# Illumina/Pisces

Hardware: AMD Instinct MI355X
Metric: candidate loci/s at 500x depth (higher is better)
Workload: dtype int32 counts + f64 likelihoods; 1 GPU; BASELINE config 2: synthetic 100000 loci x 500x amplicon pileup, SNV-only, gVCF, per GPU per step; device-resident packed tuples; depth=500, ring_batches=6, tile_loci=56, parallelism=interval-shard x1

## Files before the change

### pisces_amd/csrc/store_kernels.hip.h

```cpp
#pragma once
#include <hip/hip_runtime.h>
#include <stdint.h>
#include <type_traits>

#include "kernels.hip.h"
#include "read_walk.h"
#include "stream_kernels.hip.h"

#ifndef PISCES_ADD_OCC
#define PISCES_ADD_OCC 6
#endif
#ifdef PISCES_ADD_STAMPS
#define PISCES_STAMP(k, is_max) do { if (threadIdx.x == 0) A.stamps[(long long)blockIdx.x * 8 + ((k) == 0 ? 2 : (k) == 1 ? 3 : (k) - 2)] = (long long)wall_clock64(); } while (0)
#else
#define PISCES_STAMP(k, is_max) do { } while (0)
#endif
namespace pisces {

struct ReadDesc {
    int32_t pos0;
    uint32_t meta;
    int64_t aoff;
};
struct ReadExt {
    int64_t cig_off;
    int32_t n_cigar;
    int32_t n_bases;
};
static_assert(sizeof(ReadDesc) == 16 && sizeof(ReadExt) == 16, "descriptor layout");
constexpr uint32_t kDescLenMask = 0xFFFFFu;
constexpr uint32_t kDescComplex = 1u << 20;
constexpr uint32_t kDescReverse = 1u << 21;
constexpr uint32_t kDescGeneric = 1u << 22;
// ... 101 lines not shown
            const long long a = prev + 1, b = p;
            if (b - a > kGridGapCells || b - A.grid_base >= A.grid_n || a < A.grid_base) atomicOr(&A.state[kStateFrags], kGridBadBit);
            else { c0 = (int)(a - A.grid_base); c1 = (int)(b - A.grid_base); f0 = (int)(A.ops0 + A.cigar_offset[r]); }
        }
    }
    const bool wide = c1 - c0 >= 16;
    if (!wide)
        for (int k = c0; k <= c1; k++) A.grid[k] = f0;
    for (unsigned long long m = __ballot(wide); m != 0ull; m &= m - 1ull) {
        const int src = __builtin_ctzll(m);
        const int b0 = __builtin_amdgcn_readlane(c0, src), b1 = __builtin_amdgcn_readlane(c1, src), f = __builtin_amdgcn_readlane(f0, src);
        for (int k = b0 + lane; k <= b1; k += 64) A.grid[k] = f;
    }
    if (block == (A.n_reads - 1) / 256) {
        const int last_lane = (A.n_reads - 1) & 255;
        if ((int)(threadIdx.x >> 6) == (last_lane >> 6)) {
            const long long p_last = A.position[A.n_reads - 1];
            const long long from = max(p_last + 1 - (long long)A.grid_base, 0ll);
            for (long long k = from + lane; k < (long long)A.grid_n; k += 64) A.grid[k] = 0x7F7F7F7F;
        }
    }
}

__device__ __forceinline__ void shape_reads(const ShapeArgs& A, const int block, const bool ok)
{
    const int r = block * 256 + (int)threadIdx.x;
    int reach = 0;
    bool unsorted = false, complex_read = false, generic_read = false, has_del = false;
    if (r < A.n_reads && ok) {
        const int c0 = A.cigar_offset[r], nc = A.cigar_offset[r + 1] - c0;
        const int s0 = A.seq_offset[r], n = A.seq_offset[r + 1] - s0;
        const int32_t pos0 = A.position[r];
        int phase = 0, lead = 0;
        long long run = 0, ref_span = 0;
        bool simple = true, prev_gap = false, gap_chain = false;
        for (int c = 0; c < nc; c++) {
            const uint8_t t = A.cigar_op[c0 + c];
            const long long len = A.cigar_len[c0 + c];
            if (walk_op_ref_span(t)) ref_span += len;
            if (t == 'D' || t == 'N') { gap_chain = gap_chain || prev_gap; prev_gap = true; }
            if (t == 'M' || t == '=' || t == 'X') {
                prev_gap = false;
                if (phase == 2) simple = false;
                phase = 1;
                run += len;
            } else if (t == 'S') {
                if (phase == 0) lead += (int)len;
                else phase = 2;
            } else if (t == 'H' || t == 'P') {
                if (phase == 1 && t == 'H') phase = 2;
            } else {
                simple = false;
            }
        }
        if (run > (long long)kDescLenMask || run > n - lead) simple = false;
        ReadDesc d;
        d.pos0 = pos0;
        d.meta = (simple ? (uint32_t)run : kDescComplex) | ((A.flags[r] & 1) ? kDescReverse : 0u);
        d.aoff = A.base0 + s0 + (simple ? lead : 0);
        A.desc[A.n0 + r] = d;
        ReadExt e;
        e.cig_off = A.ops0 + c0;
        e.n_cigar = nc;
        e.n_bases = n;
        A.ext[A.n0 + r] = e;
        reach = (int)(ref_span > 0x7FFFFFFFll ? 0x7FFFFFFFll : ref_span);
        complex_read = !simple;
        bool generic = ref_span > 0xFFFFll || gap_chain;
        const long long span16 = (ref_span > 0 ? ref_span - 1 : 0) << kFragSpanShift;
        for (int c = 0; c < nc; c++) generic = generic || A.cigar_len[c0 + c] > kDescLenMask;
        if (generic) {
            d.meta |= kDescGeneric;
            A.desc[A.n0 + r] = d;
        }
        const uint8_t* const quals = A.quals + s0;
        const uint32_t rev = (A.flags[r] & 1) ? kDescReverse : 0u;
        auto dq = [&](int i) {
            const int after = quals[i], before = i > 0 ? quals[i - 1] : after;
            return before >= A.min_bq && after >= A.min_bq;
        };
        auto dir_at = [&](int i) { return A.dirs ? (uint32_t)A.dirs[s0 + i] : (rev ? (uint32_t)PISCES_DIR_REVERSE : (uint32_t)PISCES_DIR_FORWARD); };
        const bool ends_in_del = nc >= 1 && A.cigar_op[c0 + nc - 1] == 'D';
        const bool ends_in_del_soft = nc >= 2 && A.cigar_op[c0 + nc - 2] == 'D' && A.cigar_op[c0 + nc - 1] == 'S';
        int ri = 0;
        long long rp = pos0, last_mapped = (long long)pos0 - 1;
        for (int c = 0; c < nc; c++) {
            const uint8_t t = A.cigar_op[c0 + c];
            const int len = (int)A.cigar_len[c0 + c];
            ReadDesc f;
            f.pos0 = pos0;
            f.meta = rev;
            f.aoff = A.base0 + s0;
            if (!generic && len > 0) {
                if (t == 'M' || t == '=' || t == 'X') {
                    const int have = max(min(len, n - ri), 0);
                    f.meta |= (uint32_t)have;
                    f.aoff = (A.base0 + s0 + ri) | span16 | ((rp - pos0) << kFragDeltaShift);
                } else if (t == 'D' || t == 'N') {
                    int idx = -1, first = (int)(rp - pos0), count = len;
                    uint32_t dir = 0;
                    {
                        int rj = ri;
                        for (int k = c + 1; k < nc && idx < 0; k++) {
                            const uint8_t tk = A.cigar_op[c0 + k];
                            const int lk = (int)A.cigar_len[c0 + k];
                            if ((tk == 'M' || tk == '=' || tk == 'X') && lk > 0) idx = rj;
                            else if (walk_op_read_span(tk)) rj += lk;
                        }
                    }
                    bool counted = false, terminal = false;
                    if (idx >= 0 && idx < n) {
                        counted = dq(idx);
                        dir = dir_at(idx);
                    } else if (t == 'D' && c == nc - 1 && ends_in_del && n > 0) {
                        counted = dq(n - 1);
                        dir = dir_at(n - 1);
                        first = (int)(last_mapped + 1 - pos0);
                        terminal = true;
                    } else if (t == 'D' && c == nc - 2 && ends_in_del_soft) {
                        const int at = n - (int)A.cigar_len[c0 + nc - 1];
                        if (at >= 0 && at < n) {
                            counted = dq(at);
                            dir = dir_at(at);
                            first = (int)(last_mapped + 1 - pos0);
                            terminal = true;
                        }
                    }
                    if (counted && first >= 0 && first <= 0xFFFF) {
                        f.meta = rev | kFragDeletion | (uint32_t)count | (dir << kFragDirShift) | (terminal ? kFragTerminal : 0u);
                        f.aoff = (A.base0 + s0) | span16 | ((long long)first << kFragDeltaShift);
                        has_del = true;
                    }
                }
            }
            A.frag[A.ops0 + c0 + c] = f;
            if (walk_op_ref_span(t)) {
                if (walk_op_read_span(t) && len > 0) last_mapped = rp + len - 1;
                rp += len;
            }
            if (walk_op_read_span(t)) ri += len;
        }
        generic_read = generic;
        if (r > 0) unsorted = A.position[r - 1] > pos0;
        else if (A.n0 > 0) unsorted = A.desc[A.n0 - 1].pos0 > pos0;
    }
#pragma unroll
    for (int d = 32; d >= 1; d >>= 1) reach = max(reach, __shfl_xor(reach, d, 64));
    const bool any_unsorted = __ballot(unsorted) != 0ull, any_complex = __ballot(complex_read) != 0ull;
    const int frag_bits = (__ballot(generic_read) != 0ull ? 1 : 0) | (__ballot(has_del) != 0ull ? 2 : 0);
    if ((threadIdx.x & 63) == 0) {
        if (reach > A.state[kStateReach]) atomicMax(&A.state[kStateReach], reach);
        if (any_unsorted && A.state[kStateUnsorted] == 0) atomicOr(&A.state[kStateUnsorted], 1);
        if (any_complex && A.state[kStateComplex] == 0) atomicOr(&A.state[kStateComplex], 1);
        if (frag_bits & ~A.state[kStateFrags]) atomicOr(&A.state[kStateFrags], frag_bits);
    }
}
__global__ __launch_bounds__(256) void read_shape_kernel(ShapeArgs A)
{
    if ((int)blockIdx.x >= A.shape_blocks) {
        const int b = (int)blockIdx.x - A.shape_blocks;
        if (b < A.enc_blocks) encode_rows(A, b, A.enc_blocks);
        else grid_cells(A, b - A.enc_blocks);
        return;
    }
    shape_reads(A, (int)blockIdx.x, true);
}

enum { kPrepPositionNotPositive = 1, kPrepMalformed = 2, kPrepCigarMismatch = 3, kPrepPastInt32 = 4, kPrepBadDeletionDirection = 5, kPrepBadDirection = 6 };
struct PrepareArgs {
    const int32_t* position;
    const int32_t* cigar_offset;
    const uint8_t* cigar_op;
    const uint32_t* cigar_len;
    const int32_t* seq_offset;
    const uint8_t* quals;
    const uint8_t* del_dirs;
    int32_t n_reads, min_bq, block_size, count_indels;
    int64_t n_ops_total, n_bases_total;
    uint32_t* block_bits;
    int64_t n_block_bits;
    int64_t map_stride;
    int32_t* n_found;
    int32_t* n_pool;
    unsigned long long* first_error;
    int32_t* key_span;
};
constexpr int kPrepReplicas = 32;
__device__ __forceinline__ void set_keys(const PrepareArgs& A, int replica, int64_t a, int64_t b)
{
    uint32_t* const map = A.block_bits + (int64_t)(replica & (kPrepReplicas - 1)) * A.map_stride;
    for (int64_t k = a; k <= b; k++) {
        if (k >= A.n_block_bits) continue;
        const uint32_t bit = 1u << (k & 31);
        uint32_t* const w = &map[k >> 5];
        (void)__hip_atomic_fetch_or(w, bit, __ATOMIC_RELAXED, __HIP_MEMORY_SCOPE_AGENT);
    }
}
__device__ __forceinline__ long long prep_shfl64(long long v, int src_lane)
{
    const int lo = __shfl((int)(v & 0xFFFFFFFFll), src_lane, 64);
    const int hi = __shfl((int)(v >> 32), src_lane, 64);
    return ((long long)hi << 32) | (unsigned int)lo;
}
__device__ __forceinline__ void prepare_reads(const PrepareArgs& A, const int block, int& found_out, int& pool_out, bool& ok_out)
{
    constexpr int kRunSlots = 32;
    __shared__ int s_klo, s_khi, s_plo, s_eqx, s_nruns;
    __shared__ long long s_run_a[kRunSlots], s_run_b[kRunSlots];
    if (threadIdx.x == 0) { s_klo = 0x7FFFFFFF; s_khi = 0; s_plo = 0x7FFFFFFF; s_eqx = 0; s_nruns = 0; }
    __syncthreads();
    const int r = block * 256 + (int)threadIdx.x;
    found_out = pool_out = 0;
    ok_out = false;
    int k_lo = 0x7FFFFFFF, k_hi = 0, p_lo = 0x7FFFFFFF;
    int64_t run_a = 1, run_b = 0;
    bool eqx = false;
    if (r < A.n_reads) {
        int code = 0;
        p_lo = A.position[r];
        const int64_t c0 = A.cigar_offset[r], c1 = A.cigar_offset[r + 1], s0 = A.seq_offset[r], s1 = A.seq_offset[r + 1];
        const int32_t pos0 = A.position[r];
        const int64_t nc = c1 - c0, n = s1 - s0;
        int found = 0, pool = 0;
        if (c0 < 0 || c1 < c0 || c1 > A.n_ops_total || s0 < 0 || s1 < s0 || s1 > A.n_bases_total) code = kPrepMalformed;
        else if (pos0 <= 0) code = kPrepPositionNotPositive;
        if (!code) {
            const uint8_t* const quals = A.quals + s0;
            auto delq = [&](int64_t idx) {
                if (n == 0) return false;
                const int after = idx < n ? quals[idx] : quals[idx - 1];
                const int before = idx > 0 ? quals[idx - 1] : after;
                return before >= A.min_bq && after >= A.min_bq;
            };
            auto touch = [&](int64_t from, int64_t to) {
                if (to < 1) return;
                if (from < 1) from = 1;
                const int64_t a = (from + A.block_size - 1) / A.block_size, b = (to + A.block_size - 1) / A.block_size;
                if (run_b < run_a) { run_a = a; run_b = b; }
                else if (a <= run_b + 1 && b >= run_a - 1) { run_a = min(run_a, a); run_b = max(run_b, b); }
                else { set_keys(A, block, run_a, run_b); run_a = a; run_b = b; }
                k_lo = min(k_lo, (int)a);
                k_hi = max(k_hi, (int)min(b, (int64_t)0x7FFFFFFF));
            };
            int64_t read_span = 0, ref_span = 0;
            bool bad_del_dir = false;
            for (int64_t c = 0; c < nc && !code; c++) {
                const uint8_t t = A.cigar_op[c0 + c];
                const uint32_t len = A.cigar_len[c0 + c];
                if (len > 0x0FFFFFFFu) code = kPrepMalformed;
                if (walk_op_read_span(t)) read_span += len;
                if (walk_op_ref_span(t)) ref_span += len;
                if (A.del_dirs && t == 'D')
                    for (int k = 0; k < 2; k++) {
                        const uint8_t d = A.del_dirs[2 * (c0 + c) + k];
                        if (d > 2 && d != PISCES_DIR_UNTRACKED) bad_del_dir = true;
                    }
                if (A.count_indels) {
                    if (t == 'I' || t == 'D') found++;
                    if (t == 'I' && len > 32u) pool += (int)len;
                    if (t == 'X' || t == '=') eqx = true;
                }
            }
            if (!code && nc > 0 && read_span != n) code = kPrepCigarMismatch;
            if (!code && (int64_t)pos0 + ref_span > 0x7FFFFFFFll) code = kPrepPastInt32;
            if (!code && bad_del_dir) code = kPrepBadDeletionDirection;
            if (!code) {
                int64_t rp = pos0, last_mapped = (int64_t)pos0 - 1, ri = 0;
                for (int64_t c = 0; c < nc; c++) {
                    const uint8_t t = A.cigar_op[c0 + c];
                    const int64_t len = A.cigar_len[c0 + c];
                    if (walk_op_read_span(t) && walk_op_ref_span(t) && len > 0) {
                        if (rp > last_mapped + 1 && ri < n && delq(ri)) touch(last_mapped + 1, rp - 1);
                        touch(rp, rp + len - 1);
                        last_mapped = rp + len - 1;
                    }
                    if (walk_op_ref_span(t)) rp += len;
                    if (walk_op_read_span(t)) ri += len;
                }
                const bool ends_del = nc >= 1 && A.cigar_op[c0 + nc - 1] == 'D';
                const bool ends_del_soft = nc >= 2 && A.cigar_op[c0 + nc - 2] == 'D' && A.cigar_op[c0 + nc - 1] == 'S';
                if (ends_del && n > 0 && delq(n - 1)) touch(last_mapped + 1, last_mapped + (int64_t)A.cigar_len[c0 + nc - 1]);
                if (ends_del_soft) {
                    const int64_t idx = n - (int64_t)A.cigar_len[c0 + nc - 1];
                    if (idx >= 0 && idx < n && delq(idx)) touch(last_mapped + 1, last_mapped + (int64_t)A.cigar_len[c0 + nc - 2]);
                }
            }
        }
        found_out = code ? 0 : found;
        pool_out = code ? 0 : pool;
        ok_out = code == 0;
        if (code) atomicMin(A.first_error, (unsigned long long)r * 8ull + (unsigned long long)code);
    }
    {
        unsigned long long todo = __ballot(run_b >= run_a);
        const int lane = threadIdx.x & 63;
        while (todo) {
            const int l0 = __builtin_ctzll(todo);
            const long long a0 = prep_shfl64((long long)run_a, l0), b0 = prep_shfl64((long long)run_b, l0);
            const unsigned long long same = __ballot(run_b >= run_a && run_a == a0 && run_b == b0);
            if (lane == l0) {
                const int slot = atomicAdd(&s_nruns, 1);
                if (slot < kRunSlots) { s_run_a[slot] = a0; s_run_b[slot] = b0; }
                else set_keys(A, block, a0, b0);
            }
            todo &= ~same;
        }
    }
#pragma unroll
    for (int d = 32; d >= 1; d >>= 1) {
        k_lo = min(k_lo, __shfl_xor(k_lo, d, 64));
        k_hi = max(k_hi, __shfl_xor(k_hi, d, 64));
        p_lo = min(p_lo, __shfl_xor(p_lo, d, 64));
    }
    const bool any_eqx = __ballot(eqx) != 0ull;
// ... 101 lines not shown
    int32_t do_shape;
    int32_t read_blocks, stream_blocks, misc_blocks;
    const uint8_t* s_bases;
    const uint8_t* s_quals;
    const uint8_t* s_dirs;
    uint8_t* d_bases;
    uint8_t* d_quals;
    uint8_t* d_dirs;
    uint8_t* d_codes;
    int64_t n_seq;
    uint32_t enc_min_bq;
    CopyRanges16 C;
    unsigned long long* scan_state;
    unsigned int* done;
    long long* totals;
    PrepVerdict* verdict;
    int32_t* keys_out;
    int32_t capacity;
    int32_t* bad_direction;
    int32_t seq;
    long long* stamps;
};
constexpr int kAddCopiedWord = 1;
__device__ __forceinline__ void wave_wait_vmem() { asm volatile("s_waitcnt vmcnt(0)" ::: "memory"); }
constexpr int kScanDirectBlocks = 4096;
constexpr unsigned long long kScanAggregate = 1ull << 62, kScanInclusive = 2ull << 62, kScanField = 0x7FFFFFFFull;

__device__ __forceinline__ void add_stream_roles(const AddFusedArgs& A, const int sb)
{
        if (sb < A.stream_blocks) {
            PISCES_STAMP(0, false);
            const uint32_t qk4 = (0x7Fu + A.enc_min_bq) * 0x01010101u;
            const int64_t n16 = A.n_seq >> 4;
            bool bad_dir = false;
            constexpr int kStreamPieces = 4;
            for (int64_t i0 = (int64_t)sb * (256 * kStreamPieces); i0 < n16; i0 += (int64_t)A.stream_blocks * (256 * kStreamPieces)) {
                uint32_t bw[kStreamPieces][4], qw[kStreamPieces][4];
#pragma unroll
                for (int p = 0; p < kStreamPieces; p++) {
                    const int64_t i = min(i0 + p * 256 + (int64_t)threadIdx.x, n16 - 1);
                    __builtin_memcpy(bw[p], A.s_bases + 16 * i, 16);
                    __builtin_memcpy(qw[p], A.s_quals + 16 * i, 16);
                }
#pragma unroll
                for (int p = 0; p < kStreamPieces; p++) {
                    const int64_t i = i0 + p * 256 + (int64_t)threadIdx.x;
                    if (i >= n16) continue;
                    if (A.s_dirs) {
                        uint32_t dw[4];
                        __builtin_memcpy(dw, A.s_dirs + 16 * i, 16);
#pragma unroll
                        for (int k = 0; k < 4; k++) bad_dir = bad_dir || ((dw[k] + 0x7D7D7D7Du) | dw[k]) & 0x80808080u;
                        if (A.d_dirs) __builtin_memcpy(A.d_dirs + 16 * i, dw, 16);
                    }
                    if (A.d_bases) {
                        __builtin_memcpy(A.d_bases + 16 * i, bw[p], 16);
                        __builtin_memcpy(A.d_quals + 16 * i, qw[p], 16);
                    }
// ... 38 lines not shown
    if (b >= A.read_blocks) {
        add_stream_roles(A, b - A.read_blocks);
        if (A.d_bases && !A.s_dirs) {
            wave_wait_vmem();
            __syncthreads();
            if (threadIdx.x == 0) {
                unsigned int* const copied = A.done + (1 + kPrepReplicas);
                const unsigned sb = (unsigned)(b - A.read_blocks), n_wg = (unsigned)(A.stream_blocks + A.misc_blocks);
                const unsigned cls = sb & (kPrepReplicas - 1u);
                const unsigned members = (n_wg - cls + kPrepReplicas - 1u) / kPrepReplicas;
                if (__hip_atomic_fetch_add(&copied[1 + cls], 1u, __ATOMIC_RELAXED, __HIP_MEMORY_SCOPE_AGENT) == members - 1u) {
                    __hip_atomic_store(&copied[1 + cls], 0u, __ATOMIC_RELAXED, __HIP_MEMORY_SCOPE_AGENT);
                    const unsigned classes = min(n_wg, (unsigned)kPrepReplicas);
                    if (__hip_atomic_fetch_add(&copied[0], 1u, __ATOMIC_RELAXED, __HIP_MEMORY_SCOPE_AGENT) == classes - 1u) {
                        __hip_atomic_store(&copied[0], 0u, __ATOMIC_RELAXED, __HIP_MEMORY_SCOPE_AGENT);
                        __hip_atomic_store(&A.bad_direction[kAddCopiedWord], A.seq, __ATOMIC_RELAXED, __HIP_MEMORY_SCOPE_SYSTEM);
                    }
                }
            }
        }
        return;
    }
    {
    int found, pool;
    bool ok;
    PISCES_STAMP(2, false);
    PISCES_STAMP(3, true);
    prepare_reads(A.P, b, found, pool, ok);
    PISCES_STAMP(4, true);
    if (A.do_shape) shape_reads(A.S, b, ok);
    PISCES_STAMP(5, true);
    const int lane = threadIdx.x & 63, wave = threadIdx.x >> 6;
    int incl_f = found, incl_p = pool;
#pragma unroll
    for (int d = 1; d < 64; d <<= 1) {
        const int uf = __shfl_up(incl_f, d, 64), up = __shfl_up(incl_p, d, 64);
        if (lane >= d) { incl_f += uf; incl_p += up; }
    }
    if (lane == 63) { s_wf[wave] = incl_f; s_wp[wave] = incl_p; }
    __syncthreads();
    int off_f = 0, off_p = 0, agg_f = 0, agg_p = 0;
#pragma unroll
    for (int w = 0; w < 4; w++) {
        if (w < wave) { off_f += s_wf[w]; off_p += s_wp[w]; }
        agg_f += s_wf[w]; agg_p += s_wp[w];
    }
    if (wave == 0) {
        const unsigned long long mine = ((unsigned long long)(unsigned)agg_p << 31) | (unsigned long long)(unsigned)agg_f;
        long long excl_f = 0, excl_p = 0;
        if (A.read_blocks <= kScanDirectBlocks) {
            if (lane == 0) __hip_atomic_store(&A.scan_state[b], kScanAggregate | mine, __ATOMIC_RELAXED, __HIP_MEMORY_SCOPE_AGENT);
            for (int i0 = 0; i0 < b; i0 += 64 * 16) {
                unsigned long long w[16];
                for (;;) {
                    bool all = true;
// ... 25 lines not shown
                if (none & upto) { __builtin_amdgcn_s_sleep(1); continue; }
                int f = (lane <= first_incl) ? (int)(w & kScanField) : 0, p = (lane <= first_incl) ? (int)((w >> 31) & kScanField) : 0;
#pragma unroll
                for (int d = 32; d >= 1; d >>= 1) { f += __shfl_xor(f, d, 64); p += __shfl_xor(p, d, 64); }
                excl_f += f; excl_p += p;
                if (first_incl < 64) break;
                base -= 64;
            }
            if (lane == 0)
                __hip_atomic_store(&A.scan_state[b], kScanInclusive | ((unsigned long long)(excl_p + agg_p) << 31) | (unsigned long long)(excl_f + agg_f), __ATOMIC_RELAXED,
                                   __HIP_MEMORY_SCOPE_AGENT);
        }
        if (lane == 0) {
            s_excl[0] = (int)excl_f; s_excl[1] = (int)excl_p;
            if (b == A.read_blocks - 1) {
                __hip_atomic_store(&A.totals[0], excl_f + agg_f, __ATOMIC_RELAXED, __HIP_MEMORY_SCOPE_AGENT);
                __hip_atomic_store(&A.totals[1], excl_p + agg_p, __ATOMIC_RELAXED, __HIP_MEMORY_SCOPE_AGENT);
            }
        }
    }
    __syncthreads();
    PISCES_STAMP(6, true);
    if (A.P.n_found) {
        const int r = b * 256 + (int)threadIdx.x;
        if (r < A.P.n_reads) {
            A.P.n_found[r] = s_excl[0] + off_f + incl_f - found;
            A.P.n_pool[r] = s_excl[1] + off_p + incl_p - pool;
        }
        if (b == A.read_blocks - 1 && threadIdx.x == 0) { A.P.n_found[A.P.n_reads] = s_excl[0] + agg_f; A.P.n_pool[A.P.n_reads] = s_excl[1] + agg_p; }
    }
    }
    wave_wait_vmem();
    __syncthreads();
    if (threadIdx.x == 0) {
        const unsigned cls = (unsigned)b & (kPrepReplicas - 1u);
        const unsigned members = ((unsigned)A.read_blocks - cls + kPrepReplicas - 1u) / kPrepReplicas;
        int last = 0;
        if (__hip_atomic_fetch_add(&A.done[1 + cls], 1u, __ATOMIC_RELAXED, __HIP_MEMORY_SCOPE_AGENT) == members - 1u) {
            const unsigned classes = min((unsigned)A.read_blocks, (unsigned)kPrepReplicas);
            last = __hip_atomic_fetch_add(&A.done[0], 1u, __ATOMIC_RELAXED, __HIP_MEMORY_SCOPE_AGENT) == classes - 1u;
        }
        s_last = last;
    }
    __syncthreads();
    PISCES_STAMP(7, true);
    if (!s_last) return;
    prepare_collect(A.P.block_bits, A.P.map_stride, A.P.key_span, A.P.first_error, A.totals, A.verdict, A.keys_out, A.capacity);
    __syncthreads();
    for (int i = threadIdx.x; i < A.read_blocks; i += 256) A.scan_state[i] = 0ull;
    if (threadIdx.x < kPrepReplicas) {
// ... 740 lines not shown
```

### pisces_amd/csrc/surface_store.inc.h

```cpp

static int32_t store_run_deferred(PiscesHip* h)
{
    if (h->deferred_grid.empty()) return PISCES_OK;
    for (auto& d : h->deferred_grid) hipLaunchKernelGGL(read_shape_kernel, dim3(d.blocks), dim3(256), 0, h->stream, d.S);
    h->deferred_grid.clear();
    PISCES_HIP_CHECK(h, hipGetLastError());
    return PISCES_OK;
}

static void store_view(PiscesHip* h, StoreView* V)
{
    (void)store_run_deferred(h);
    std::memset(V, 0, sizeof(*V));
    int n = 0;
    for (auto& sp : h->segments) {
        const ReadSegment& g = *sp;
        if (g.n_reads == 0 || n == kMaxSegments) continue;
        SegmentView& v = V->seg[n++];
        v.frag = g.frag.p;
        v.desc = g.desc.p;
        v.ext = g.ext.p;
        v.bases = g.v_bases;
        v.quals = g.v_quals;
        v.codes = g.v_codes;
// ... 365 lines not shown
    const int64_t n_block_bits = (0x7FFFFFFFll + bs - 1) / bs + 2;
    if (n_block_bits > (1ll << 27)) return fail(h, PISCES_E_UNSUPPORTED, "add_reads: a batch on the device needs a block size of 16 positions or more");
    const size_t map_words = (size_t)((n_block_bits + 31) / 32);
    const size_t map_copies = map_words * kPrepReplicas * sizeof(uint32_t) > (32u << 20) ? 1 : (size_t)kPrepReplicas;
    const size_t map_stride = map_copies == 1 ? 0 : map_words;
    if (h->prep_map_copies != map_copies) h->prep_map_clean = false;
    h->prep_map_copies = map_copies;
    { const size_t before = h->d_prep_map.cap; PISCES_HIP_CHECK(h, h->d_prep_map.reserve(map_words * map_copies)); if (h->d_prep_map.cap != before) h->prep_map_clean = false; }
    PISCES_HIP_CHECK(h, h->d_found_pool_first.reserve((size_t)nr + 1));
    if (!h->prep_map_clean) {
        PISCES_HIP_CHECK(h, hipMemsetAsync(h->d_prep_map.p, 0, map_words * map_copies * sizeof(uint32_t), h->stream));
        h->prep_map_clean = true;
    }
    constexpr size_t kWordsSpan = 0, kWordsError = 4 * kPrepReplicas * sizeof(int32_t), kWordsDone = kWordsError + 8, kWordsTotals = kWordsDone + 8 * (2 * (1 + kPrepReplicas) * 4 / 8 + 1), kWordsBytes = kWordsTotals + 16;
    if (!h->d_fused_words.p) {
        PISCES_HIP_CHECK(h, h->d_fused_words.reserve(kWordsBytes));
        uint8_t init[kWordsBytes];
        std::memset(init, 0, sizeof(init));
        int32_t* sp = (int32_t*)init;
        for (int r = 0; r < kPrepReplicas; r++) { sp[4 * r] = 0x7FFFFFFF; sp[4 * r + 1] = 0; sp[4 * r + 2] = 0x7FFFFFFF; sp[4 * r + 3] = 0; }
        std::memset(init + kWordsError, 0xFF, 8);
        { int32_t rcu = meta_upload(h, h->d_fused_words.p, init, sizeof(init)); if (rcu) return rcu; }
    }
    const int32_t read_blocks = (nr + 255) / 256;
    {
        const size_t before = h->d_fused_scan.cap;
        PISCES_HIP_CHECK(h, h->d_fused_scan.reserve((size_t)read_blocks + 1));
        if (h->d_fused_scan.cap != before) PISCES_HIP_CHECK(h, hipMemsetAsync(h->d_fused_scan.p, 0, h->d_fused_scan.cap * sizeof(unsigned long long), h->stream));
    }
    if (!h->h_prep) PISCES_HIP_CHECK(h, host_alloc((void**)&h->h_prep, kPrepBytes));
    PrepVerdict* const verdict = (PrepVerdict*)h->h_prep;
    int32_t* const keys = prep_keys(h);
    int32_t* const bad_direction = prep_stream_words(h);
    *bad_direction = 0;
    bad_direction[kAddCopiedWord] = 0;
    AddFusedArgs F;
    std::memset(&F, 0, sizeof(F));
    PrepareArgs& A = F.P;
    A.position = src ? src->position : (const int32_t*)(d + L.off_pos);
    A.cigar_offset = src ? src->cigar_offset : (const int32_t*)(d + L.off_coff);
    A.cigar_op = src ? src->cigar_op : d + L.off_cop;
    A.cigar_len = src ? src->cigar_len : (const uint32_t*)(d + L.off_clen);
    A.seq_offset = src ? src->seq_offset : (const int32_t*)(d + L.off_soff);
    A.quals = src ? src->quals : d + L.off_quals;
    A.del_dirs = has_deldirs ? (src ? src->deletion_directions : d + L.off_deldirs) : nullptr;
    A.n_reads = nr; A.min_bq = h->cfg.min_base_call_quality; A.block_size = bs; A.count_indels = count_indels ? 1 : 0;
    A.n_ops_total = (int64_t)n_cig; A.n_bases_total = (int64_t)n_seq;
// ... 11 lines not shown
        }
        F.d_codes = shape->enc_codes;
    }
    F.s_bases = src ? src->bases : d + L.off_bases;
    F.s_quals = src ? src->quals : d + L.off_quals;
    F.s_dirs = has_dirs ? (src ? src->directions : d + L.off_dirs) : nullptr;
    if (src) { F.d_bases = d + L.off_bases; F.d_quals = d + L.off_quals; F.d_dirs = has_dirs ? d + L.off_dirs : nullptr; }
    F.n_seq = (int64_t)n_seq;
    F.enc_min_bq = (uint32_t)std::min(std::max(h->cfg.min_base_call_quality, 0), 127);
    int64_t misc_bytes = 0;
    if (src) {
        int k = 0;
        auto range = [&](size_t off, const void* from, size_t bytes) { F.C.dst[k] = d + off; F.C.src[k] = (const uint8_t*)from; F.C.n[k] = (int64_t)bytes; misc_bytes = std::max<int64_t>(misc_bytes, (int64_t)bytes); k++; };
        range(L.off_pos, src->position, (size_t)nr * 4);
        range(L.off_flags, src->flags, (size_t)nr);
        range(L.off_coff, src->cigar_offset, ((size_t)nr + 1) * 4);
        range(L.off_cop, src->cigar_op, n_cig);
        range(L.off_clen, src->cigar_len, n_cig * 4);
        range(L.off_soff, src->seq_offset, ((size_t)nr + 1) * 4);
        if (has_deldirs) range(L.off_deldirs, src->deletion_directions, 2 * n_cig);
    }
    F.read_blocks = read_blocks;
    const bool stream = n_seq > 0 && (src || F.d_codes || has_dirs);
    F.stream_blocks = stream ? (int32_t)std::min<int64_t>(((int64_t)n_seq + 4 * 16 * 256 - 1) / (4 * 16 * 256), 16384) : 0;
    F.misc_blocks = src ? (int32_t)std::min<int64_t>(std::max<int64_t>((misc_bytes / 16 + 255) / 256, 1), 64) : 0;
    F.scan_state = h->d_fused_scan.p;
    F.done = (unsigned int*)(h->d_fused_words.p + kWordsDone);
    F.totals = (long long*)(h->d_fused_words.p + kWordsTotals);
    F.verdict = verdict;
    F.keys_out = keys;
    F.capacity = kPrepKeys;
    F.bad_direction = bad_direction;
    if (++h->fused_seq <= 0) h->fused_seq = 1;
    F.seq = h->fused_seq;
    verdict->ready = 0;
#ifdef PISCES_ADD_STAMPS
    const size_t n_wg = (size_t)(F.read_blocks + F.stream_blocks + F.misc_blocks);
    PISCES_HIP_CHECK(h, h->d_add_stamps.reserve(n_wg * 8));
    PISCES_HIP_CHECK(h, hipMemsetAsync(h->d_add_stamps.p, 0, n_wg * 8 * sizeof(long long), h->stream));
    PISCES_HIP_CHECK(h, hipStreamSynchronize(h->stream));
    F.stamps = h->d_add_stamps.p;
#endif
    h->chain_have[0] = false;
    h->chain_add_open = false;
    if (h->chain_timing && src) { PISCES_HIP_CHECK(h, hipEventRecord(h->ev_chain[0], h->stream)); h->chain_add_open = true; }
    hipLaunchKernelGGL(add_fused_kernel, dim3((unsigned)(F.read_blocks + F.stream_blocks + F.misc_blocks)), dim3(256), 0, h->stream, F);
    PISCES_HIP_CHECK(h, hipGetLastError());
// ... 541 lines not shown
```

Measured before the change: 2.656 billion candidate loci/s.

## Process four reads per lane in fused add kernel with batched cigar walks

The fused read-add kernel now has each thread handle several consecutive reads. prepare_reads and shape_reads are templated on the reads-per-lane count, and their CIGAR walks run in lockstep with the loads batched ahead of use. This gives more independent memory loads in flight per thread, and the host launches correspondingly fewer read blocks. The occupancy hint drops from 6 to 3 and the stream pieces per block go from 4 to 8. The trade is higher register pressure and more divergence when CIGAR lengths differ across the reads handled by one lane.

```diff
diff --git a/pisces_amd/csrc/store_kernels.hip.h b/pisces_amd/csrc/store_kernels.hip.h
--- a/pisces_amd/csrc/store_kernels.hip.h
+++ b/pisces_amd/csrc/store_kernels.hip.h
@@ -7,8 +7,14 @@
 #include "read_walk.h"
 #include "stream_kernels.hip.h"
 
+#ifndef PISCES_ADD_READS_PER_LANE
+#define PISCES_ADD_READS_PER_LANE 4
+#endif
 #ifndef PISCES_ADD_OCC
-#define PISCES_ADD_OCC 6
+#define PISCES_ADD_OCC 3
+#endif
+#ifndef PISCES_ADD_STREAM_PIECES
+#define PISCES_ADD_STREAM_PIECES 8
 #endif
 #ifdef PISCES_ADD_STAMPS
 #define PISCES_STAMP(k, is_max) do { if (threadIdx.x == 0) A.stamps[(long long)blockIdx.x * 8 + ((k) == 0 ? 2 : (k) == 1 ? 3 : (k) - 2)] = (long long)wall_clock64(); } while (0)
@@ -156,127 +162,196 @@
     }
 }
 
-__device__ __forceinline__ void shape_reads(const ShapeArgs& A, const int block, const bool ok)
-{
-    const int r = block * 256 + (int)threadIdx.x;
+template <int R>
+__device__ __forceinline__ void shape_reads(const ShapeArgs& A, const int block, const bool (&ok)[R])
+{
+    const int64_t r0 = ((int64_t)block * 256 + (int64_t)threadIdx.x) * R;
+    const int64_t last = (int64_t)A.n_reads - 1;
     int reach = 0;
     bool unsorted = false, complex_read = false, generic_read = false, has_del = false;
-    if (r < A.n_reads && ok) {
-        const int c0 = A.cigar_offset[r], nc = A.cigar_offset[r + 1] - c0;
-        const int s0 = A.seq_offset[r], n = A.seq_offset[r + 1] - s0;
-        const int32_t pos0 = A.position[r];
-        int phase = 0, lead = 0;
-        long long run = 0, ref_span = 0;
-        bool simple = true, prev_gap = false, gap_chain = false;
-        for (int c = 0; c < nc; c++) {
-            const uint8_t t = A.cigar_op[c0 + c];
-            const long long len = A.cigar_len[c0 + c];
-            if (walk_op_ref_span(t)) ref_span += len;
-            if (t == 'D' || t == 'N') { gap_chain = gap_chain || prev_gap; prev_gap = true; }
-            if (t == 'M' || t == '=' || t == 'X') {
-                prev_gap = false;
-                if (phase == 2) simple = false;
-                phase = 1;
-                run += len;
-            } else if (t == 'S') {
-                if (phase == 0) lead += (int)len;
-                else phase = 2;
-            } else if (t == 'H' || t == 'P') {
-                if (phase == 1 && t == 'H') phase = 2;
+    int32_t co[R + 1], so[R + 1], pos[R];
+    uint8_t flg[R];
+    bool go[R];
+#pragma unroll
+    for (int k = 0; k <= R; k++) {
+        const int64_t i = min(r0 + k, last + 1);
+        co[k] = A.cigar_offset[i];
+        so[k] = A.seq_offset[i];
+    }
+#pragma unroll
+    for (int k = 0; k < R; k++) {
+        const int64_t i = min(r0 + k, last);
+        pos[k] = A.position[i];
+        flg[k] = A.flags[i];
+        go[k] = r0 + k <= last && ok[k];
+    }
+    bool have_prev = false;
+    int32_t prev_pos = 0;
+    if (r0 <= last) {
+        if (r0 > 0) { have_prev = true; prev_pos = A.position[r0 - 1]; }
+        else if (A.n0 > 0) { have_prev = true; prev_pos = A.desc[A.n0 - 1].pos0; }
+    }
+    int nc[R], n[R], maxc = 0;
+#pragma unroll
+    for (int k = 0; k < R; k++) {
+        nc[k] = go[k] ? co[k + 1] - co[k] : 0;
+        n[k] = so[k + 1] - so[k];
+        maxc = max(maxc, nc[k]);
+    }
+    int phase[R], lead[R];
+    long long run[R], ref_span_k[R];
+    bool simple[R], prev_gap[R], gap_chain_k[R], generic_k[R];
+    uint8_t t_last[R];
+    uint32_t len_last[R];
+#pragma unroll
+    for (int k = 0; k < R; k++) { phase[k] = 0; lead[k] = 0; run[k] = 0; ref_span_k[k] = 0; simple[k] = true; prev_gap[k] = gap_chain_k[k] = generic_k[k] = false; t_last[k] = 0; len_last[k] = 0; }
+    long long span16[R];
+    uint32_t rev[R];
+#pragma unroll
+    for (int k = 0; k < R; k++) { span16[k] = 0; rev[k] = (flg[k] & 1) ? kDescReverse : 0u; }
+    for (int c = 0; c < maxc; c++) {
+        uint8_t t[R];
+        uint32_t ln[R];
+#pragma unroll
+        for (int k = 0; k < R; k++) {
+            const int64_t i = c < nc[k] ? (int64_t)co[k] + c : 0;
+            t[k] = A.cigar_op[i];
+            ln[k] = A.cigar_len[i];
+        }
+#pragma unroll
+        for (int k = 0; k < R; k++) {
+            if (c >= nc[k]) continue;
+            const uint8_t tk = t[k];
+            const long long len = ln[k];
+            if (walk_op_ref_span(tk)) ref_span_k[k] += len;
+            if (tk == 'D' || tk == 'N') { gap_chain_k[k] = gap_chain_k[k] || prev_gap[k]; prev_gap[k] = true; }
+            if (tk == 'M' || tk == '=' || tk == 'X') {
+                prev_gap[k] = false;
+                if (phase[k] == 2) simple[k] = false;
+                phase[k] = 1;
+                run[k] += len;
+            } else if (tk == 'S') {
+                if (phase[k] == 0) lead[k] += (int)len;
+                else phase[k] = 2;
+            } else if (tk == 'H' || tk == 'P') {
+                if (phase[k] == 1 && tk == 'H') phase[k] = 2;
             } else {
-                simple = false;
-            }
-        }
-        if (run > (long long)kDescLenMask || run > n - lead) simple = false;
+                simple[k] = false;
+            }
+            generic_k[k] = generic_k[k] || ln[k] > kDescLenMask;
+            if (c == nc[k] - 1) { t_last[k] = tk; len_last[k] = ln[k]; }
+        }
+    }
+#pragma unroll
+    for (int k = 0; k < R; k++) {
+        if (!go[k]) continue;
+        const int64_t r = r0 + k;
+        if (run[k] > (long long)kDescLenMask || run[k] > n[k] - lead[k]) simple[k] = false;
+        const long long ref_span = ref_span_k[k];
+        const bool gap_chain = gap_chain_k[k];
+        bool generic = ref_span > 0xFFFFll || gap_chain;
+        generic_k[k] = generic = generic || generic_k[k];
         ReadDesc d;
-        d.pos0 = pos0;
-        d.meta = (simple ? (uint32_t)run : kDescComplex) | ((A.flags[r] & 1) ? kDescReverse : 0u);
-        d.aoff = A.base0 + s0 + (simple ? lead : 0);
+        d.pos0 = pos[k];
+        d.meta = (simple[k] ? (uint32_t)run[k] : kDescComplex) | rev[k] | (generic_k[k] ? kDescGeneric : 0u);
+        d.aoff = A.base0 + so[k] + (simple[k] ? lead[k] : 0);
         A.desc[A.n0 + r] = d;
         ReadExt e;
-        e.cig_off = A.ops0 + c0;
-        e.n_cigar = nc;
-        e.n_bases = n;
+        e.cig_off = A.ops0 + co[k];
+        e.n_cigar = nc[k];
+        e.n_bases = n[k];
         A.ext[A.n0 + r] = e;
-        reach = (int)(ref_span > 0x7FFFFFFFll ? 0x7FFFFFFFll : ref_span);
-        complex_read = !simple;
-        bool generic = ref_span > 0xFFFFll || gap_chain;
-        const long long span16 = (ref_span > 0 ? ref_span - 1 : 0) << kFragSpanShift;
-        for (int c = 0; c < nc; c++) generic = generic || A.cigar_len[c0 + c] > kDescLenMask;
-        if (generic) {
-            d.meta |= kDescGeneric;
-            A.desc[A.n0 + r] = d;
-        }
-        const uint8_t* const quals = A.quals + s0;
-        const uint32_t rev = (A.flags[r] & 1) ? kDescReverse : 0u;
-        auto dq = [&](int i) {
-            const int after = quals[i], before = i > 0 ? quals[i - 1] : after;
-            return before >= A.min_bq && after >= A.min_bq;
-        };
-        auto dir_at = [&](int i) { return A.dirs ? (uint32_t)A.dirs[s0 + i] : (rev ? (uint32_t)PISCES_DIR_REVERSE : (uint32_t)PISCES_DIR_FORWARD); };
-        const bool ends_in_del = nc >= 1 && A.cigar_op[c0 + nc - 1] == 'D';
-        const bool ends_in_del_soft = nc >= 2 && A.cigar_op[c0 + nc - 2] == 'D' && A.cigar_op[c0 + nc - 1] == 'S';
-        int ri = 0;
-        long long rp = pos0, last_mapped = (long long)pos0 - 1;
-        for (int c = 0; c < nc; c++) {
-            const uint8_t t = A.cigar_op[c0 + c];
-            const int len = (int)A.cigar_len[c0 + c];
+        reach = max(reach, (int)(ref_span_k[k] > 0x7FFFFFFFll ? 0x7FFFFFFFll : ref_span_k[k]));
+        complex_read = complex_read || !simple[k];
+        generic_read = generic_read || generic_k[k];
+        span16[k] = (ref_span_k[k] > 0 ? ref_span_k[k] - 1 : 0) << kFragSpanShift;
+        unsorted = unsorted || (k == 0 ? have_prev && prev_pos > pos[0] : pos[k > 0 ? k - 1 : 0] > pos[k]);
+    }
+    int ri[R];
+    long long rp[R], last_mapped[R];
+#pragma unroll
+    for (int k = 0; k < R; k++) { ri[k] = 0; rp[k] = pos[k]; last_mapped[k] = (long long)pos[k] - 1; }
+    for (int c = 0; c < maxc; c++) {
+        uint8_t t[R];
+        int ln[R];
+#pragma unroll
+        for (int k = 0; k < R; k++) {
+            const int64_t i = c < nc[k] ? (int64_t)co[k] + c : 0;
+            t[k] = A.cigar_op[i];
+            ln[k] = (int)A.cigar_len[i];
+        }
+        int qi[R], first_k[R];
+        bool want_q[R], terminal[R];
+#pragma unroll
+        for (int k = 0; k < R; k++) {
+            want_q[k] = terminal[k] = false;
+            qi[k] = 0;
+            first_k[k] = (int)(rp[k] - pos[k]);
+            if (c >= nc[k] || generic_k[k] || ln[k] <= 0 || !(t[k] == 'D' || t[k] == 'N')) continue;
+            int idx = -1;
+            {
+                int rj = ri[k];
+                for (int j = c + 1; j < nc[k] && idx < 0; j++) {
+                    const uint8_t tj = A.cigar_op[(int64_t)co[k] + j];
+                    const int lj = (int)A.cigar_len[(int64_t)co[k] + j];
+                    if ((tj == 'M' || tj == '=' || tj == 'X') && lj > 0) idx = rj;
+                    else if (walk_op_read_span(tj)) rj += lj;
+                }
+            }
+            if (idx >= 0 && idx < n[k]) {
+                qi[k] = idx;
+                want_q[k] = true;
+            } else if (t[k] == 'D' && c == nc[k] - 1 && n[k] > 0) {
+                qi[k] = n[k] - 1;
+                want_q[k] = terminal[k] = true;
+            } else if (t[k] == 'D' && c == nc[k] - 2 && t_last[k] == 'S') {
+                const int at = n[k] - (int)len_last[k];
+                if (at >= 0 && at < n[k]) { qi[k] = at; want_q[k] = terminal[k] = true; }
+            }
+            if (terminal[k]) first_k[k] = (int)(last_mapped[k] + 1 - pos[k]);
+        }
+        int q_after[R], q_before[R];
+        uint32_t dir[R];
+#pragma unroll
+        for (int k = 0; k < R; k++) {
+            q_after[k] = q_before[k] = 0;
+            dir[k] = rev[k] ? (uint32_t)PISCES_DIR_REVERSE : (uint32_t)PISCES_DIR_FORWARD;
+            if (!want_q[k]) continue;
+            q_after[k] = A.quals[(int64_t)so[k] + qi[k]];
+            q_before[k] = A.quals[(int64_t)so[k] + (qi[k] > 0 ? qi[k] - 1 : qi[k])];
+            if (A.dirs) dir[k] = A.dirs[(int64_t)so[k] + qi[k]];
+        }
+#pragma unroll
+        for (int k = 0; k < R; k++) {
+            if (c >= nc[k]) continue;
+            const uint8_t tk = t[k];
+            const int len = ln[k];
             ReadDesc f;
-            f.pos0 = pos0;
-            f.meta = rev;
-            f.aoff = A.base0 + s0;
-            if (!generic && len > 0) {
-                if (t == 'M' || t == '=' || t == 'X') {
-                    const int have = max(min(len, n - ri), 0);
+            f.pos0 = pos[k];
+            f.meta = rev[k];
+            f.aoff = A.base0 + so[k];
+            if (!generic_k[k] && len > 0) {
+                if (tk == 'M' || tk == '=' || tk == 'X') {
+                    const int have = max(min(len, n[k] - ri[k]), 0);
                     f.meta |= (uint32_t)have;
-                    f.aoff = (A.base0 + s0 + ri) | span16 | ((rp - pos0) << kFragDeltaShift);
-                } else if (t == 'D' || t == 'N') {
-                    int idx = -1, first = (int)(rp - pos0), count = len;
-                    uint32_t dir = 0;
-                    {
-                        int rj = ri;
-                        for (int k = c + 1; k < nc && idx < 0; k++) {
-                            const uint8_t tk = A.cigar_op[c0 + k];
-                            const int lk = (int)A.cigar_len[c0 + k];
-                            if ((tk == 'M' || tk == '=' || tk == 'X') && lk > 0) idx = rj;
-                            else if (walk_op_read_span(tk)) rj += lk;
-                        }
-                    }
-                    bool counted = false, terminal = false;
-                    if (idx >= 0 && idx < n) {
-                        counted = dq(idx);
-                        dir = dir_at(idx);
-                    } else if (t == 'D' && c == nc - 1 && ends_in_del && n > 0) {
-                        counted = dq(n - 1);
-                        dir = dir_at(n - 1);
-                        first = (int)(last_mapped + 1 - pos0);
-                        terminal = true;
-                    } else if (t == 'D' && c == nc - 2 && ends_in_del_soft) {
-                        const int at = n - (int)A.cigar_len[c0 + nc - 1];
-                        if (at >= 0 && at < n) {
-                            counted = dq(at);
-                            dir = dir_at(at);
-                            first = (int)(last_mapped + 1 - pos0);
-                            terminal = true;
-                        }
-                    }
+                    f.aoff = (A.base0 + so[k] + ri[k]) | span16[k] | ((rp[k] - pos[k]) << kFragDeltaShift);
+                } else if (want_q[k]) {
+                    const bool counted = q_before[k] >= A.min_bq && q_after[k] >= A.min_bq;
+                    const int first = first_k[k];
                     if (counted && first >= 0 && first <= 0xFFFF) {
-                        f.meta = rev | kFragDeletion | (uint32_t)count | (dir << kFragDirShift) | (terminal ? kFragTerminal : 0u);
-                        f.aoff = (A.base0 + s0) | span16 | ((long long)first << kFragDeltaShift);
+                        f.meta = rev[k] | kFragDeletion | (uint32_t)len | (dir[k] << kFragDirShift) | (terminal[k] ? kFragTerminal : 0u);
+                        f.aoff = (A.base0 + so[k]) | span16[k] | ((long long)first << kFragDeltaShift);
                         has_del = true;
                     }
                 }
             }
-            A.frag[A.ops0 + c0 + c] = f;
-            if (walk_op_ref_span(t)) {
-                if (walk_op_read_span(t) && len > 0) last_mapped = rp + len - 1;
-                rp += len;
-            }
-            if (walk_op_read_span(t)) ri += len;
-        }
-        generic_read = generic;
-        if (r > 0) unsorted = A.position[r - 1] > pos0;
-        else if (A.n0 > 0) unsorted = A.desc[A.n0 - 1].pos0 > pos0;
+            A.frag[A.ops0 + co[k] + c] = f;
+            if (walk_op_ref_span(tk)) {
+                if (walk_op_read_span(tk) && len > 0) last_mapped[k] = rp[k] + len - 1;
+                rp[k] += len;
+            }
+            if (walk_op_read_span(tk)) ri[k] += len;
+        }
     }
 #pragma unroll
     for (int d = 32; d >= 1; d >>= 1) reach = max(reach, __shfl_xor(reach, d, 64));
@@ -297,7 +372,8 @@
         else grid_cells(A, b - A.enc_blocks);
         return;
     }
-    shape_reads(A, (int)blockIdx.x, true);
+    const bool ok[1] = {true};
+    shape_reads<1>(A, (int)blockIdx.x, ok);
 }
 
 enum { kPrepPositionNotPositive = 1, kPrepMalformed = 2, kPrepCigarMismatch = 3, kPrepPastInt32 = 4, kPrepBadDeletionDirection = 5, kPrepBadDirection = 6 };
@@ -336,94 +412,173 @@
     const int hi = __shfl((int)(v >> 32), src_lane, 64);
     return ((long long)hi << 32) | (unsigned int)lo;
 }
-__device__ __forceinline__ void prepare_reads(const PrepareArgs& A, const int block, int& found_out, int& pool_out, bool& ok_out)
+template <int R>
+__device__ __forceinline__ void prepare_reads(const PrepareArgs& A, const int block, int (&found_out)[R], int (&pool_out)[R], bool (&ok_out)[R])
 {
     constexpr int kRunSlots = 32;
     __shared__ int s_klo, s_khi, s_plo, s_eqx, s_nruns;
     __shared__ long long s_run_a[kRunSlots], s_run_b[kRunSlots];
     if (threadIdx.x == 0) { s_klo = 0x7FFFFFFF; s_khi = 0; s_plo = 0x7FFFFFFF; s_eqx = 0; s_nruns = 0; }
     __syncthreads();
-    const int r = block * 256 + (int)threadIdx.x;
-    found_out = pool_out = 0;
-    ok_out = false;
+    const int64_t r0 = ((int64_t)block * 256 + (int64_t)threadIdx.x) * R;
+    const int64_t last = (int64_t)A.n_reads - 1;
     int k_lo = 0x7FFFFFFF, k_hi = 0, p_lo = 0x7FFFFFFF;
     int64_t run_a = 1, run_b = 0;
     bool eqx = false;
-    if (r < A.n_reads) {
-        int code = 0;
-        p_lo = A.position[r];
-        const int64_t c0 = A.cigar_offset[r], c1 = A.cigar_offset[r + 1], s0 = A.seq_offset[r], s1 = A.seq_offset[r + 1];
-        const int32_t pos0 = A.position[r];
-        const int64_t nc = c1 - c0, n = s1 - s0;
-        int found = 0, pool = 0;
-        if (c0 < 0 || c1 < c0 || c1 > A.n_ops_total || s0 < 0 || s1 < s0 || s1 > A.n_bases_total) code = kPrepMalformed;
-        else if (pos0 <= 0) code = kPrepPositionNotPositive;
-        if (!code) {
-            const uint8_t* const quals = A.quals + s0;
-            auto delq = [&](int64_t idx) {
-                if (n == 0) return false;
-                const int after = idx < n ? quals[idx] : quals[idx - 1];
-                const int before = idx > 0 ? quals[idx - 1] : after;
-                return before >= A.min_bq && after >= A.min_bq;
-            };
-            auto touch = [&](int64_t from, int64_t to) {
-                if (to < 1) return;
-                if (from < 1) from = 1;
-                const int64_t a = (from + A.block_size - 1) / A.block_size, b = (to + A.block_size - 1) / A.block_size;
-                if (run_b < run_a) { run_a = a; run_b = b; }
-                else if (a <= run_b + 1 && b >= run_a - 1) { run_a = min(run_a, a); run_b = max(run_b, b); }
-                else { set_keys(A, block, run_a, run_b); run_a = a; run_b = b; }
-                k_lo = min(k_lo, (int)a);
-                k_hi = max(k_hi, (int)min(b, (int64_t)0x7FFFFFFF));
-            };
-            int64_t read_span = 0, ref_span = 0;
-            bool bad_del_dir = false;
-            for (int64_t c = 0; c < nc && !code; c++) {
-                const uint8_t t = A.cigar_op[c0 + c];
-                const uint32_t len = A.cigar_len[c0 + c];
-                if (len > 0x0FFFFFFFu) code = kPrepMalformed;
-                if (walk_op_read_span(t)) read_span += len;
-                if (walk_op_ref_span(t)) ref_span += len;
-                if (A.del_dirs && t == 'D')
-                    for (int k = 0; k < 2; k++) {
-                        const uint8_t d = A.del_dirs[2 * (c0 + c) + k];
-                        if (d > 2 && d != PISCES_DIR_UNTRACKED) bad_del_dir = true;
-                    }
-                if (A.count_indels) {
-                    if (t == 'I' || t == 'D') found++;
-                    if (t == 'I' && len > 32u) pool += (int)len;
-                    if (t == 'X' || t == '=') eqx = true;
+    int32_t co[R + 1], so[R + 1], pos[R];
+#pragma unroll
+    for (int k = 0; k <= R; k++) {
+        const int64_t i = min(r0 + k, last + 1);
+        co[k] = A.cigar_offset[i];
+        so[k] = A.seq_offset[i];
+    }
+#pragma unroll
+    for (int k = 0; k < R; k++) pos[k] = A.position[min(r0 + k, last)];
+    int code[R], nc[R], found[R], pool[R], maxc = 0;
+    int64_t n[R];
+#pragma unroll
+    for (int k = 0; k < R; k++) {
+        const bool valid = r0 + k <= last;
+        const int64_t c0 = co[k], c1 = co[k + 1], s0 = so[k], s1 = so[k + 1];
+        code[k] = 0;
+        found[k] = pool[k] = 0;
+        if (valid) {
+            p_lo = min(p_lo, pos[k]);
+            if (c0 < 0 || c1 < c0 || c1 > A.n_ops_total || s0 < 0 || s1 < s0 || s1 > A.n_bases_total) code[k] = kPrepMalformed;
+            else if (pos[k] <= 0) code[k] = kPrepPositionNotPositive;
+        }
+        nc[k] = valid && !code[k] ? (int)(c1 - c0) : 0;
+        n[k] = s1 - s0;
+        maxc = max(maxc, nc[k]);
+    }
+    int64_t read_span[R], ref_span[R];
+    bool bad_del_dir[R];
+    uint8_t t_last[R], t_prev[R];
+    uint32_t len_last[R], len_prev[R];
+#pragma unroll
+    for (int k = 0; k < R; k++) { read_span[k] = ref_span[k] = 0; bad_del_dir[k] = false; t_last[k] = t_prev[k] = 0; len_last[k] = len_prev[k] = 0; }
+    for (int c = 0; c < maxc; c++) {
+        uint8_t t[R];
+        uint32_t ln[R];
+        bool act[R];
+#pragma unroll
+        for (int k = 0; k < R; k++) {
+            act[k] = c < nc[k] && !code[k];
+            const int64_t i = act[k] ? (int64_t)co[k] + c : 0;
+            t[k] = A.cigar_op[i];
+            ln[k] = A.cigar_len[i];
+        }
+#pragma unroll
+        for (int k = 0; k < R; k++) {
+            if (!act[k]) continue;
+            const uint8_t tk = t[k];
+            const uint32_t len = ln[k];
+            if (len > 0x0FFFFFFFu) code[k] = kPrepMalformed;
+            if (walk_op_read_span(tk)) read_span[k] += len;
+            if (walk_op_ref_span(tk)) ref_span[k] += len;
+            if (A.del_dirs && tk == 'D')
+                for (int j = 0; j < 2; j++) {
+                    const uint8_t d = A.del_dirs[2 * ((int64_t)co[k] + c) + j];
+                    if (d > 2 && d != PISCES_DIR_UNTRACKED) bad_del_dir[k] = true;
                 }
-            }
-            if (!code && nc > 0 && read_span != n) code = kPrepCigarMismatch;
-            if (!code && (int64_t)pos0 + ref_span > 0x7FFFFFFFll) code = kPrepPastInt32;
-            if (!code && bad_del_dir) code = kPrepBadDeletionDirection;
-            if (!code) {
-                int64_t rp = pos0, last_mapped = (int64_t)pos0 - 1, ri = 0;
-                for (int64_t c = 0; c < nc; c++) {
-                    const uint8_t t = A.cigar_op[c0 + c];
-                    const int64_t len = A.cigar_len[c0 + c];
-                    if (walk_op_read_span(t) && walk_op_ref_span(t) && len > 0) {
-                        if (rp > last_mapped + 1 && ri < n && delq(ri)) touch(last_mapped + 1, rp - 1);
-                        touch(rp, rp + len - 1);
-                        last_mapped = rp + len - 1;
-                    }
-                    if (walk_op_ref_span(t)) rp += len;
-                    if (walk_op_read_span(t)) ri += len;
-                }
-                const bool ends_del = nc >= 1 && A.cigar_op[c0 + nc - 1] == 'D';
-                const bool ends_del_soft = nc >= 2 && A.cigar_op[c0 + nc - 2] == 'D' && A.cigar_op[c0 + nc - 1] == 'S';
-                if (ends_del && n > 0 && delq(n - 1)) touch(last_mapped + 1, last_mapped + (int64_t)A.cigar_len[c0 + nc - 1]);
-                if (ends_del_soft) {
-                    const int64_t idx = n - (int64_t)A.cigar_len[c0 + nc - 1];
-                    if (idx >= 0 && idx < n && delq(idx)) touch(last_mapped + 1, last_mapped + (int64_t)A.cigar_len[c0 + nc - 2]);
-                }
-            }
-        }
-        found_out = code ? 0 : found;
-        pool_out = code ? 0 : pool;
-        ok_out = code == 0;
-        if (code) atomicMin(A.first_error, (unsigned long long)r * 8ull + (unsigned long long)code);
+            if (A.count_indels) {
+                if (tk == 'I' || tk == 'D') found[k]++;
+                if (tk == 'I' && len > 32u) pool[k] += (int)len;
+                if (tk == 'X' || tk == '=') eqx = true;
+            }
+            if (c == nc[k] - 2) { t_prev[k] = tk; len_prev[k] = len; }
+            if (c == nc[k] - 1) { t_last[k] = tk; len_last[k] = len; }
+        }
+    }
+    bool go[R];
+    int maxg = 0;
+#pragma unroll
+    for (int k = 0; k < R; k++) {
+        const bool valid = r0 + k <= last;
+        if (valid && !code[k]) {
+            if (nc[k] > 0 && read_span[k] != n[k]) code[k] = kPrepCigarMismatch;
+            else if ((int64_t)pos[k] + ref_span[k] > 0x7FFFFFFFll) code[k] = kPrepPastInt32;
+            else if (bad_del_dir[k]) code[k] = kPrepBadDeletionDirection;
+        }
+        go[k] = valid && !code[k];
+        if (go[k]) maxg = max(maxg, nc[k]);
+    }
+    auto touch = [&](int64_t from, int64_t to) {
+        if (to < 1) return;
+        if (from < 1) from = 1;
+        const int64_t a = (from + A.block_size - 1) / A.block_size, b = (to + A.block_size - 1) / A.block_size;
+        if (run_b < run_a) { run_a = a; run_b = b; }
+        else if (a <= run_b + 1 && b >= run_a - 1) { run_a = min(run_a, a); run_b = max(run_b, b); }
+        else { set_keys(A, block, run_a, run_b); run_a = a; run_b = b; }
+        k_lo = min(k_lo, (int)a);
+        k_hi = max(k_hi, (int)min(b, (int64_t)0x7FFFFFFF));
+    };
+    auto delq_after = [&](int64_t idx, int64_t nn) { return idx < nn ? idx : idx - 1; };
+    auto delq_before = [&](int64_t idx, int64_t nn) { return idx > 0 ? idx - 1 : (idx < nn ? idx : idx - 1); };
+    int64_t rp[R], last_mapped[R], ri[R];
+#pragma unroll
+    for (int k = 0; k < R; k++) { rp[k] = pos[k]; last_mapped[k] = (int64_t)pos[k] - 1; ri[k] = 0; }
+    for (int c = 0; c < maxg; c++) {
+        uint8_t t[R];
+        int64_t ln[R];
+        bool act[R], aligned[R], need[R];
+#pragma unroll
+        for (int k = 0; k < R; k++) {
+            act[k] = go[k] && c < nc[k];
+            const int64_t i = act[k] ? (int64_t)co[k] + c : 0;
+            t[k] = A.cigar_op[i];
+            ln[k] = A.cigar_len[i];
+        }
+        int q_after[R], q_before[R];
+#pragma unroll
+        for (int k = 0; k < R; k++) {
+            aligned[k] = act[k] && walk_op_read_span(t[k]) && walk_op_ref_span(t[k]) && ln[k] > 0;
+            need[k] = aligned[k] && rp[k] > last_mapped[k] + 1 && ri[k] < n[k];
+            q_after[k] = q_before[k] = 0;
+            if (need[k]) {
+                q_after[k] = A.quals[so[k] + delq_after(ri[k], n[k])];
+                q_before[k] = A.quals[so[k] + delq_before(ri[k], n[k])];
+            }
+        }
+#pragma unroll
+        for (int k = 0; k < R; k++) {
+            if (!act[k]) continue;
+            if (aligned[k]) {
+                if (need[k] && q_before[k] >= A.min_bq && q_after[k] >= A.min_bq) touch(last_mapped[k] + 1, rp[k] - 1);
+                touch(rp[k], rp[k] + ln[k] - 1);
+                last_mapped[k] = rp[k] + ln[k] - 1;
+            }
+            if (walk_op_ref_span(t[k])) rp[k] += ln[k];
+            if (walk_op_read_span(t[k])) ri[k] += ln[k];
+        }
+    }
+    {
+        bool need[R];
+        int64_t at[R], del_len[R];
+        int q_after[R], q_before[R];
+#pragma unroll
+        for (int k = 0; k < R; k++) {
+            const bool ends_del = go[k] && nc[k] >= 1 && t_last[k] == 'D';
+            const bool ends_del_soft = go[k] && nc[k] >= 2 && t_prev[k] == 'D' && t_last[k] == 'S';
+            at[k] = ends_del ? n[k] - 1 : n[k] - (int64_t)len_last[k];
+            del_len[k] = ends_del ? (int64_t)len_last[k] : (int64_t)len_prev[k];
+            need[k] = (ends_del && n[k] > 0) || (ends_del_soft && at[k] >= 0 && at[k] < n[k]);
+            q_after[k] = q_before[k] = 0;
+            if (need[k]) {
+                q_after[k] = A.quals[so[k] + delq_after(at[k], n[k])];
+                q_before[k] = A.quals[so[k] + delq_before(at[k], n[k])];
+            }
+        }
+#pragma unroll
+        for (int k = 0; k < R; k++)
+            if (need[k] && q_before[k] >= A.min_bq && q_after[k] >= A.min_bq) touch(last_mapped[k] + 1, last_mapped[k] + del_len[k]);
+    }
+#pragma unroll
+    for (int k = 0; k < R; k++) {
+        found_out[k] = code[k] ? 0 : found[k];
+        pool_out[k] = code[k] ? 0 : pool[k];
+        ok_out[k] = go[k];
+        if (code[k]) atomicMin(A.first_error, (unsigned long long)(r0 + k) * 8ull + (unsigned long long)code[k]);
     }
     {
         unsigned long long todo = __ballot(run_b >= run_a);
@@ -571,6 +726,8 @@
     long long* stamps;
 };
 constexpr int kAddCopiedWord = 1;
+constexpr int kAddReadsPerLane = PISCES_ADD_READS_PER_LANE;
+constexpr int kStreamPieces = PISCES_ADD_STREAM_PIECES;
 __device__ __forceinline__ void wave_wait_vmem() { asm volatile("s_waitcnt vmcnt(0)" ::: "memory"); }
 constexpr int kScanDirectBlocks = 4096;
 constexpr unsigned long long kScanAggregate = 1ull << 62, kScanInclusive = 2ull << 62, kScanField = 0x7FFFFFFFull;
@@ -582,7 +739,6 @@
             const uint32_t qk4 = (0x7Fu + A.enc_min_bq) * 0x01010101u;
             const int64_t n16 = A.n_seq >> 4;
             bool bad_dir = false;
-            constexpr int kStreamPieces = 4;
             for (int64_t i0 = (int64_t)sb * (256 * kStreamPieces); i0 < n16; i0 += (int64_t)A.stream_blocks * (256 * kStreamPieces)) {
                 uint32_t bw[kStreamPieces][4], qw[kStreamPieces][4];
 #pragma unroll
@@ -667,15 +823,19 @@
         return;
     }
     {
-    int found, pool;
-    bool ok;
+    constexpr int R = kAddReadsPerLane;
+    int found_k[R], pool_k[R];
+    bool ok[R];
     PISCES_STAMP(2, false);
     PISCES_STAMP(3, true);
-    prepare_reads(A.P, b, found, pool, ok);
+    prepare_reads<R>(A.P, b, found_k, pool_k, ok);
     PISCES_STAMP(4, true);
-    if (A.do_shape) shape_reads(A.S, b, ok);
+    if (A.do_shape) shape_reads<R>(A.S, b, ok);
     PISCES_STAMP(5, true);
     const int lane = threadIdx.x & 63, wave = threadIdx.x >> 6;
+    int found = 0, pool = 0;
+#pragma unroll
+    for (int k = 0; k < R; k++) { found += found_k[k]; pool += pool_k[k]; }
     int incl_f = found, incl_p = pool;
 #pragma unroll
     for (int d = 1; d < 64; d <<= 1) {
@@ -747,10 +907,13 @@
     __syncthreads();
     PISCES_STAMP(6, true);
     if (A.P.n_found) {
-        const int r = b * 256 + (int)threadIdx.x;
-        if (r < A.P.n_reads) {
-            A.P.n_found[r] = s_excl[0] + off_f + incl_f - found;
-            A.P.n_pool[r] = s_excl[1] + off_p + incl_p - pool;
+        const int64_t r0 = ((int64_t)b * 256 + (int64_t)threadIdx.x) * R;
+        int at_f = s_excl[0] + off_f + incl_f - found, at_p = s_excl[1] + off_p + incl_p - pool;
+#pragma unroll
+        for (int k = 0; k < R; k++) {
+            if (r0 + k < (int64_t)A.P.n_reads) { A.P.n_found[r0 + k] = at_f; A.P.n_pool[r0 + k] = at_p; }
+            at_f += found_k[k];
+            at_p += pool_k[k];
         }
         if (b == A.read_blocks - 1 && threadIdx.x == 0) { A.P.n_found[A.P.n_reads] = s_excl[0] + agg_f; A.P.n_pool[A.P.n_reads] = s_excl[1] + agg_p; }
     }
diff --git a/pisces_amd/csrc/surface_store.inc.h b/pisces_amd/csrc/surface_store.inc.h
--- a/pisces_amd/csrc/surface_store.inc.h
+++ b/pisces_amd/csrc/surface_store.inc.h
@@ -411,7 +411,7 @@
         std::memset(init + kWordsError, 0xFF, 8);
         { int32_t rcu = meta_upload(h, h->d_fused_words.p, init, sizeof(init)); if (rcu) return rcu; }
     }
-    const int32_t read_blocks = (nr + 255) / 256;
+    const int32_t read_blocks = (int32_t)(((int64_t)nr + 256 * kAddReadsPerLane - 1) / (256 * kAddReadsPerLane));
     {
         const size_t before = h->d_fused_scan.cap;
         PISCES_HIP_CHECK(h, h->d_fused_scan.reserve((size_t)read_blocks + 1));
@@ -469,7 +469,7 @@
     }
     F.read_blocks = read_blocks;
     const bool stream = n_seq > 0 && (src || F.d_codes || has_dirs);
-    F.stream_blocks = stream ? (int32_t)std::min<int64_t>(((int64_t)n_seq + 4 * 16 * 256 - 1) / (4 * 16 * 256), 16384) : 0;
+    F.stream_blocks = stream ? (int32_t)std::min<int64_t>(((int64_t)n_seq + kStreamPieces * 16 * 256 - 1) / (kStreamPieces * 16 * 256), 16384) : 0;
     F.misc_blocks = src ? (int32_t)std::min<int64_t>(std::max<int64_t>((misc_bytes / 16 + 255) / 256, 1), 64) : 0;
     F.scan_state = h->d_fused_scan.p;
     F.done = (unsigned int*)(h->d_fused_words.p + kWordsDone);
```

Result: no change. 2.650 billion candidate loci/s (-0.2%).
